# vribeiro1/artspeech

Measured on AMD Instinct MI355X. Metric: articulator-frames/sec (fwd+bwd), higher is better.
Workload: dtype f32

## Files before the change

artspeech_amd/csrc/artspeech.hip:

```cpp
#include <stdlib.h>

#include <algorithm>
#include <mutex>
#include <vector>

#include "gemm_internal.h"
#include "rowops.h"

namespace {

constexpr int D = AS_HEAD_HIDDEN;
constexpr int64_t SLAB_FLOATS = 16LL << 20;
constexpr int64_t SLAB2_FLOATS = 28LL << 20;

struct Carve {
    int64_t off = 0;
    int64_t take(int64_t n) {
        const int64_t o = off;
        off += as_round_up(n, 64);
        return o;
    }
};

struct HeadWs {
// ... 115 lines not shown
    as_gemm g{};
    g.A = A; g.B = Bm; g.C = C; g.M = M; g.N = N; g.K = K;
    g.a_i = 1; g.a_k = lda; g.b_j = 1; g.b_k = ldb; g.ldc = ldc;
    g.batch = batch; g.a_batch = ab; g.b_batch = bb; g.c_batch = cb; g.b_kshift = kshift; g.b_kT = kT; g.b_kshift_batch = kshift_batch;
    g.splitk_ws = slab; g.splitk_ws_floats = SLAB_FLOATS; g.colsum = colsum; g.colsum_batch = csb; g.cu_budget = cu_budget;
    return as_gemm_f32(&g, st);
}

int head_fold(const as_dims& d, const as_layout& L, const float* P, int64_t rows, float* ws, hipStream_t st) {
    const int A = d.n_art, H = d.hidden, O = 2 * d.n_samp;
    const HeadWs w = head_ws(d, rows);
    AS_STEP("head.fold", st, as_fold(P + L.w1, P + L.ln1_g, P + L.ln1_b, P + L.b1, ws + w.w1f, ws + w.b1f, A, D, H, st));
    AS_STEP("head.fold", st, as_fold(P + L.w2, P + L.ln2_g, P + L.ln2_b, P + L.b2, ws + w.w2f, ws + w.b2f, A, D, D, st));
    AS_STEP("head.fold", st, as_fold(P + L.w3, P + L.ln3_g, P + L.ln3_b, P + L.b3, ws + w.w3f, ws + w.b3f, A, O, D, st, (int)as_round_up(O, 32)));
    {
        const int Opad = (int)as_round_up(O, 32), Hp = (int)as_round_up(H, 32);
        auto up = [&](int64_t off) { return reinterpret_cast<uint16_t*>(ws + off); };
        as_planes_job j[6] = {
            {ws + w.w1f, H, 1, (long)D * H, A, D, H, D, Hp, up(w.w1p)},
            {ws + w.w2f, D, 1, (long)D * D, A, D, D, D, D, up(w.w2p)},
            {ws + w.w3f, D, 1, (long)Opad * D, A, O, D, (int)as_round_up(O, OUT_BN), D, up(w.w3p)},
            {ws + w.w2f, 1, D, (long)D * D, A, D, D, D, D, up(w.w2tp)},
            {ws + w.w3f, 1, D, (long)Opad * D, A, D, O, D, Opad, up(w.w3tp)},
            {ws + w.w1f, 1, H, 0, 1, H, A * D, (int)as_round_up(H, 128), A * D, up(w.w1tp)},
        };
        AS_STEP("head.planes", st, as_emit_planes(j, 6, st));
    }
    return 0;
}

struct Criterion { const float* tgt; long tgt_T; const int* lengths; int T; float scale; float* loss; float* dout; };

int head_fwd_impl(const as_dims& d, const as_layout& L, const float* P, const float* x, int64_t rows, float* out, float* ws,
                  hipStream_t st, const Criterion* crit = nullptr) {
    (void)P;
    const int A = d.n_art, H = d.hidden, O = 2 * d.n_samp;
    const HeadWs w = head_ws(d, rows);
    const int R = (int)rows;
    AS_STEP("head.norm0", st, as_normalize_fwd(x, ws + w.xhat, ws + w.rstd0, rows, H, st));
    const long AD = (long)A * D;
    const int Opad = (int)as_round_up(O, 32);
    unsigned long long* bits1 = reinterpret_cast<unsigned long long*>(ws + w.bits1);
    unsigned long long* bits2 = reinterpret_cast<unsigned long long*>(ws + w.bits2);
    as_lin l1{};
    l1.A = ws + w.xhat; l1.lda = H; l1.a_batch = 0;
    l1.B = ws + w.w1f; l1.ldb = H; l1.b_batch = (long)D * H; l1.b_kc = 1;
    l1.C = ws + w.r1hat; l1.ldc = AD; l1.c_batch = D;
    l1.bias = ws + w.b1f; l1.bias_batch = D;
    l1.M = R; l1.N = D; l1.K = H; l1.batch = A; l1.epi = 1;
    l1.rstd = ws + w.rstd1; l1.bits = bits1;
    const uint16_t* w1p = reinterpret_cast<const uint16_t*>(ws + w.w1p);
    const uint16_t* w2p = reinterpret_cast<const uint16_t*>(ws + w.w2p);
    if (H % 32 == 0) {
        l1.Bp = w1p; l1.bp_rows = D; l1.bp_batch = as_planes_batch_stride(D, H); l1.bp_plane = A * l1.bp_batch;
    }
    int took;
    bool crit_done = false;
    {
        AS_PROF("head.gemm1", st);
        took = as_lin_try(&l1, st);
        AS_REQUIRE(took >= 0, took, "head gemm1: launch failed");
    }
    if (!took) {
        AS_STEP("head.gemm1", st, gemm_nt(ws + w.xhat, H, ws + w.w1f, H, ws + w.r1, AD, ws + w.b1f, R, A * D, H, 1, st));
        AS_STEP("head.norm1", st, as_normalize_fwd(ws + w.r1, ws + w.r1hat, ws + w.rstd1, rows * A, D, st, bits1));
    }
    as_lin l2 = l1;
    l2.A = ws + w.r1hat; l2.lda = AD; l2.a_batch = D;
    l2.B = ws + w.w2f; l2.ldb = D; l2.b_batch = (long)D * D;
    l2.C = ws + w.r2hat; l2.bias = ws + w.b2f;
    l2.K = D; l2.rstd = ws + w.rstd2; l2.bits = bits2;
    l2.Bp = w2p; l2.bp_rows = D; l2.bp_batch = as_planes_batch_stride(D, D); l2.bp_plane = A * l2.bp_batch;
// ... 17 lines not shown
        AS_PROF("head.gemm3", st);
        as_lin_out lo{};
        lo.A = ws + w.r2hat; lo.lda = AD; lo.a_batch = D;
        lo.B = ws + w.w3f; lo.ldb = D; lo.b_batch = (long)Opad * D; lo.b_rows = Opad;
        lo.bias = ws + w.b3f; lo.bias_batch = O;
        lo.out = out; lo.ldo = (long)A * O; lo.o_batch = O;
        lo.M = R; lo.N = O; lo.K = D; lo.batch = A;
        lo.Bp = reinterpret_cast<const uint16_t*>(ws + w.w3p); lo.bp_rows = (int)as_round_up(O, OUT_BN);
        lo.bp_batch = as_planes_batch_stride(lo.bp_rows, D); lo.bp_plane = A * lo.bp_batch;
        int n_part = 0;
        if (crit) {
            lo.tgt = crit->tgt; lo.tgt_T = crit->tgt_T; lo.lengths = crit->lengths; lo.T = crit->T; lo.scale = crit->scale;
            lo.dout = crit->dout; lo.partial = ws + w.lpart; lo.partial_capacity = w.lpart_n; lo.loss = crit->loss;
        }
        took = as_lin_out_try(&lo, &n_part, st);
        AS_REQUIRE(took >= 0, took, "head gemm3: launch failed");
        if (took && crit && n_part > 0) AS_TRY(as_loss_final(ws + w.lpart, n_part, crit->scale, crit->loss, st));
        crit_done = took && crit;
        if (!took) {
            took = as_lin_try(&l3, st);
            AS_REQUIRE(took >= 0, took, "head gemm3: launch failed");
        }
    }
    if (!took)
        AS_STEP("head.gemm3", st, gemm_nt(ws + w.r2hat, AD, ws + w.w3f, D, out, (long)A * O, ws + w.b3f, R, O, D, 2, st, A, D,
                       (long)Opad * D, O, O));
    if (crit && !crit_done) {
        AS_STEP("loss", st, as_euclid_masked_fwd_bwd_presigmoid(out, crit->tgt, crit->tgt_T, crit->lengths, (int32_t)(rows / crit->T), crit->T, A,
                                                               d.n_samp, crit->scale, crit->loss, crit->dout, ws + w.lpart, st));
    }
    return 0;
}

int head_bwd_dx(const as_dims& d, const as_layout& L, const float* P, const float* out, const float* dout, int64_t rows,
                float* dx, const float* relu_src, float* ws, hipStream_t st, bool presig = false) {
    (void)L; (void)P;
    const int A = d.n_art, H = d.hidden, O = 2 * d.n_samp;
    const HeadWs w = head_ws(d, rows);
    const int R = (int)rows;
    const long AD = (long)A * D, AO = (long)A * O;
    const float* dpre3 = presig ? dout : ws + w.dpre3;
    if (!presig) AS_STEP("headb.sigmoid", st, as_sigmoid_bwd(out, dout, ws + w.dpre3, rows * AO, st));
    const int Opad = (int)as_round_up(O, 32);
    const unsigned long long* bits1 = reinterpret_cast<const unsigned long long*>(ws + w.bits1);
    const unsigned long long* bits2 = reinterpret_cast<const unsigned long long*>(ws + w.bits2);
    as_lin b3{};
    b3.A = dpre3; b3.lda = AO; b3.a_batch = O;
    b3.B = ws + w.w3f; b3.ldb = D; b3.b_batch = (long)Opad * D; b3.b_kc = 0;
    b3.C = ws + w.dz2; b3.ldc = AD; b3.c_batch = D;
    b3.M = R; b3.N = D; b3.K = Opad; b3.ka_valid = O; b3.batch = A; b3.epi = 2;
    b3.xhat = ws + w.r2hat; b3.ldx = AD; b3.x_batch = D; b3.rstd_in = ws + w.rstd2; b3.bits_in = bits2;
    b3.Bp = reinterpret_cast<const uint16_t*>(ws + w.w3tp); b3.bp_rows = D; b3.bp_batch = as_planes_batch_stride(D, Opad);
    b3.bp_plane = A * b3.bp_batch;
    int took;
    {
        AS_PROF("headb.dx3", st);
        took = as_lin_try(&b3, st);
        AS_REQUIRE(took >= 0, took, "head dx3: launch failed");
    }
    if (!took) {
        AS_STEP("headb.dx3", st, gemm_nn(dpre3, AO, ws + w.w3f, D, ws + w.dz2, AD, R, D, O, st, A, O, (long)Opad * D, D));
        AS_STEP("headb.norm2", st, as_normalize_bwd(ws + w.dz2, ws + w.r2hat, ws + w.rstd2, nullptr, ws + w.dz2, rows * A, D, st, bits2));
    }
    as_lin b2 = b3;
    b2.A = ws + w.dz2; b2.lda = AD; b2.a_batch = D;
    b2.B = ws + w.w2f; b2.b_batch = (long)D * D;
    b2.C = ws + w.dz1; b2.K = D; b2.ka_valid = D;
    b2.xhat = ws + w.r1hat; b2.rstd_in = ws + w.rstd1; b2.bits_in = bits1;
    b2.Bp = reinterpret_cast<const uint16_t*>(ws + w.w2tp); b2.bp_batch = as_planes_batch_stride(D, D); b2.bp_plane = A * b2.bp_batch;
    {
        AS_PROF("headb.dx2", st);
        took = as_lin_try(&b2, st);
        AS_REQUIRE(took >= 0, took, "head dx2: launch failed");
    }
    if (!took) {
        AS_STEP("headb.dx2", st, gemm_nn(ws + w.dz2, AD, ws + w.w2f, D, ws + w.dz1, AD, R, D, D, st, A, D, (long)D * D, D));
        AS_STEP("headb.norm1", st, as_normalize_bwd(ws + w.dz1, ws + w.r1hat, ws + w.rstd1, nullptr, ws + w.dz1, rows * A, D, st, bits1));
    }
    int dx1_slabs = 0;
    if (H <= 256 && H % 4 == 0) {
        as_lin l{};
        l.A = ws + w.dz1; l.lda = AD;
        l.Bp = reinterpret_cast<const uint16_t*>(ws + w.w1tp); l.bp_rows = (int)as_round_up(H, 128);
        l.bp_batch = as_planes_batch_stride(l.bp_rows, (int)AD); l.bp_plane = l.bp_batch;
        l.C = ws + w.slab; l.ldc = H;
        l.M = R; l.N = H; l.K = (int)AD; l.batch = 1;
        const int want = (int)std::max<int64_t>(1, std::min<int64_t>(8, 512 / std::max(1, as_cdiv(R, 64))));
        const int slabs = as_lin_plain_s6_slabs((int)AD, want);
        if ((int64_t)slabs * R * H <= SLAB_FLOATS) {
            AS_PROF("headb.dx1", st);
            const int took1 = as_lin_plain_s6(&l, want, (long)R * H, st);
            AS_REQUIRE(took1 >= 0, took1, "head dx1: launch failed");
            if (took1) dx1_slabs = slabs;
        }
    }
    if (!dx1_slabs)
        AS_STEP("headb.dx1", st, gemm_nn(ws + w.dz1, AD, ws + w.w1f, H, ws + w.dxhat, H, R, H, (int)AD, st, 1, 0, 0, 0, ws + w.slab));
    AS_STEP("headb.norm0", st, as_normalize_bwd(dx1_slabs ? ws + w.slab : ws + w.dxhat, ws + w.xhat, ws + w.rstd0, relu_src, dx, rows, H, st, nullptr,
                                                 dx1_slabs ? dx1_slabs : 1, (long)R * H));
    return 0;
}

struct TrunkJob { const float* dz; const float* y; float* dW; float* db; int H; };

int head_bwd_dw(const as_dims& d, const as_layout& L, const float* P, int64_t rows, float* G, float* ws, float* slab,
                hipStream_t st, const float* dpre3_in = nullptr, int cu_budget = 0, long slab_floats = SLAB_FLOATS,
                const TrunkJob* trunk = nullptr, int part = 0, int unfold_layers = -1) {
    const int A = d.n_art, H = d.hidden, O = 2 * d.n_samp;
    const HeadWs w = head_ws(d, rows);
    const int R = (int)rows;
    const long AD = (long)A * D, AO = (long)A * O;
    const float* dpre3 = dpre3_in ? dpre3_in : ws + w.dpre3;
    as_wgrad_job jobs[4] = {};
    as_gemm& g3 = jobs[0].g;
    g3.A = dpre3; g3.a_i = 1; g3.a_k = AO; g3.a_batch = O; g3.M = O;
    g3.B = ws + w.r2hat; g3.b_j = 1; g3.b_k = AD; g3.b_batch = D; g3.N = D;
    g3.C = ws + w.dw3f; g3.ldc = D; g3.c_batch = (long)O * D; g3.K = R; g3.batch = A;
    g3.colsum = G + L.b3; g3.colsum_batch = O;
    as_gemm& g1 = jobs[1].g;
    g1 = g3;
    g1.A = ws + w.xhat; g1.a_k = H; g1.a_batch = 0; g1.M = H;
    g1.B = ws + w.dz1;
    g1.C = ws + w.dw1f; g1.ldc = H; g1.c_batch = (long)D * H;
    g1.colsum = nullptr; g1.colsum_batch = 0;
    jobs[1].colsum_b = G + L.b1; jobs[1].colsum_b_batch = D; jobs[1].c_trans = 1;
    as_wgrad_job job2{};
    as_gemm& g2 = job2.g;
    g2 = g3;
    g2.A = ws + w.dz2; g2.a_k = AD; g2.a_batch = D; g2.M = D;
    g2.B = ws + w.r1hat;
// ... 221 lines not shown

extern "C" int as_artspeech_fwd(const as_dims* d, const float* P, const int64_t* tokens, int64_t tok_stride,
                                const int32_t* lengths, int32_t B, int32_t T, float* out, float* ws, int32_t train,
                                const as_opts* opts, void* stream) {
    AS_TRY(check_dims(d, "as_artspeech_fwd"));
    const float pdrop = (opts && train) ? opts->gru_dropout : 0.f;
    AS_REQUIRE(pdrop >= 0.f && pdrop < 1.f, AS_ERR_BAD_ARG, "as_artspeech_fwd: dropout %g not in [0, 1)", (double)pdrop);
    AS_REQUIRE(P && tokens && out && ws && B > 0 && T > 0 && tok_stride >= T, AS_ERR_BAD_ARG, "as_artspeech_fwd: bad argument");
    AS_REQUIRE(d->simple || lengths, AS_ERR_BAD_ARG, "as_artspeech_fwd: lengths required for the GRU model");
    AS_REQUIRE((int64_t)B * T < (1LL << 31), AS_ERR_BAD_ARG, "as_artspeech_fwd: B*T too large");
    hipStream_t st = (hipStream_t)stream;
    as_layout L;
    AS_TRY(as_artspeech_layout(d, &L));
    const ModelWs w = model_ws(*d, B, T);
    const int V = d->vocab, E = d->embed, H = d->hidden, R = B * T;
    StreamState* sd = d->simple ? nullptr : side_for(st);
    const bool late = opts && opts->fold_wait_event;
    if (late) {
        const hipError_t e = hipStreamWaitEvent(sd ? sd->side : st, (hipEvent_t)opts->fold_wait_event, 0);
        AS_REQUIRE(e == hipSuccess, (int)e, "as_artspeech_fwd: cannot wait for fold_wait_event: %s", hipGetErrorString(e));
    }
    if (sd) {
        if (!late) AS_TRY(fork_to(st, sd->side, sd->fork[0]));
        AS_TRY(head_fold(*d, L, P, R, ws + w.head, sd->side));
        AS_TRY(as_count_bad_tokens(tokens, tok_stride, T, R, V, reinterpret_cast<int*>(ws + w.tokflag), sd->side));
        if (hipEventRecord(sd->join, sd->side) != hipSuccess) {
            as_set_error("as_artspeech_fwd: event record failed");
            return AS_ERR_BAD_ARG;
        }
    } else {
        AS_TRY(head_fold(*d, L, P, R, ws + w.head, st));
        AS_TRY(as_count_bad_tokens(tokens, tok_stride, T, R, V, reinterpret_cast<int*>(ws + w.tokflag), st));
    }
    if (!d->simple) {
        if ((long)V * E <= 16384 && ((size_t)4 * E + 64 * ((size_t)E + 1)) * sizeof(float) <= 65536)
            AS_STEP("gru.table0", st, as_token_table(P + L.embedding, P + L.w_ih[0], P + L.b_ih[0], V, 6 * H, E, ws + w.tab0, st));
        else
            AS_STEP("gru.table0", st, gemm_nt(P + L.embedding, E, P + L.w_ih[0], E, ws + w.tab0, 6 * H, P + L.b_ih[0], V, 6 * H, E, 0, st));
        AS_STEP("gru.fwd_l0", st, as_gru_bidir_fwd_tokens(ws + w.tab0, tokens, tok_stride, V, P + L.w_hh[0], P + L.b_hh[0], lengths, B, T, H, ws + w.y0,
                                train ? ws + w.g0 : nullptr, st));
        const float* l1_in = ws + w.y0;
        if (pdrop > 0.f) {
            AS_STEP("gru.dropout", st, as_dropout(ws + w.y0, ws + w.y0d, (long)R * 2 * H, pdrop, opts->dropout_seed, st));
            l1_in = ws + w.y0d;
        }
        AS_STEP("gru.xproj1", st, gemm_nt(l1_in, 2 * H, P + L.w_ih[1], 2 * H, ws + w.xp1, 6 * H, P + L.b_ih[1], R, 6 * H, 2 * H, 0, st));
        AS_STEP("gru.fwd_l1", st, as_gru_bidir_fwd(ws + w.xp1, nullptr, 0, P + L.w_hh[1], P + L.b_hh[1], lengths, B, T, H, ws + w.y1,
                                train ? ws + w.g1 : nullptr, st));
        AS_STEP("trunk.linear", st, gemm_nt(ws + w.y1, 2 * H, P + L.lin_w, 2 * H, ws + w.lin, H, P + L.lin_b, R, H, 2 * H, 1, st));
    } else if (pdrop > 0.f) {
        AS_TRY(as_gather_rows(P + L.embedding, tokens, tok_stride, T, R, E, ws + w.y0, st, V));
        AS_TRY(as_dropout(ws + w.y0, ws + w.y0, (long)R * E, pdrop, opts->dropout_seed, st));
        AS_TRY(gemm_nt(ws + w.y0, E, P + L.lin_w, E, ws + w.lin, H, P + L.lin_b, R, H, E, 1, st));
    } else {
        AS_TRY(gemm_nt(P + L.embedding, E, P + L.lin_w, E, ws + w.tab0, H, P + L.lin_b, V, H, E, 1, st));
        AS_TRY(as_gather_rows(ws + w.tab0, tokens, tok_stride, T, R, H, ws + w.lin, st, V));
    }
    if (sd && hipStreamWaitEvent(st, sd->join, 0) != hipSuccess) {
        as_set_error("as_artspeech_fwd: stream wait failed");
        return AS_ERR_BAD_ARG;
    }
    if (opts && opts->loss_targets) {
        AS_REQUIRE(train && lengths && opts->loss_out && opts->loss_dout && opts->loss_tgt_T >= T, AS_ERR_BAD_ARG,
                   "as_artspeech_fwd: fused criterion needs train, lengths, loss_out, loss_dout and loss_tgt_T >= T");
        const Criterion crit{opts->loss_targets, (long)opts->loss_tgt_T, lengths, T, opts->loss_scale, opts->loss_out, opts->loss_dout};
        return head_fwd_impl(*d, L, P, ws + w.lin, R, out, ws + w.head, st, &crit);
    }
    return head_fwd_impl(*d, L, P, ws + w.lin, R, out, ws + w.head, st);
}

extern "C" int as_artspeech_dw2(const as_dims* d, const float* P, int32_t B, int32_t T, float* G, float* ws, void* stream) {
    AS_TRY(check_dims(d, "as_artspeech_dw2"));
    AS_REQUIRE(!d->simple && P && G && ws && B > 0 && T > 0, AS_ERR_BAD_ARG, "as_artspeech_dw2: bad argument");
    as_layout L;
    AS_TRY(as_artspeech_layout(d, &L));
    const ModelWs w = model_ws(*d, B, T);
    const HeadWs hw = head_ws(*d, (int64_t)B * T);
    float* hws = ws + w.head;
    return head_bwd_dw(*d, L, P, (int64_t)B * T, G, hws, hws + hw.slab2, (hipStream_t)stream, nullptr, 192, SLAB2_FLOATS, nullptr, 2, 2);
}

extern "C" int as_artspeech_bwd(const as_dims* d, const float* P, const int64_t* tokens, int64_t tok_stride,
                                const int32_t* lengths, int32_t B, int32_t T, const float* out, const float* dout, float* G,
                                float* ws, const as_opts* opts, void* stream) {
    AS_TRY(check_dims(d, "as_artspeech_bwd"));
    const float pdrop = opts ? opts->gru_dropout : 0.f;
    AS_REQUIRE(pdrop >= 0.f && pdrop < 1.f, AS_ERR_BAD_ARG, "as_artspeech_bwd: bad dropout option");
    AS_REQUIRE(P && tokens && out && dout && G && ws && B > 0 && T > 0 && tok_stride >= T, AS_ERR_BAD_ARG,
               "as_artspeech_bwd: bad argument");
    AS_REQUIRE(d->simple || lengths, AS_ERR_BAD_ARG, "as_artspeech_bwd: lengths required for the GRU model");
    hipStream_t st = (hipStream_t)stream;
    as_layout L;
    AS_TRY(as_artspeech_layout(d, &L));
    const ModelWs w = model_ws(*d, B, T);
    const HeadWs hw = head_ws(*d, (int64_t)B * T);
    const int V = d->vocab, E = d->embed, H = d->hidden, R = B * T;
    float* slab = ws + w.head + hw.slab;
    float* slab2 = ws + w.head + hw.slab2;
    float* dzlin = ws + w.head + hw.dxhat;
    float* hws = ws + w.head;
    const bool presig = opts && opts->dout_presigmoid;
    const float* dpre3 = presig ? dout : nullptr;
    AS_TRY(head_bwd_dx(*d, L, P, out, dout, R, dzlin, ws + w.lin, hws, st, presig));
    AS_REQUIRE(!(d->simple && opts && opts->defer_dw2), AS_ERR_UNSUPPORTED, "as_artspeech_bwd: defer_dw2 is for the GRU model");
    if (d->simple) {
        AS_TRY(head_bwd_dw(*d, L, P, R, G, hws, slab, st, dpre3));
        AS_TRY(record_heads_done(st, st));
        if (pdrop > 0.f) {
            AS_TRY(gemm_tn(dzlin, H, ws + w.y0, E, G + L.lin_w, E, H, E, R, st, slab, G + L.lin_b, 0));
            AS_TRY(gemm_nn(dzlin, H, P + L.lin_w, E, ws + w.dy0, E, R, E, H, st));
            AS_TRY(as_dropout(ws + w.dy0, ws + w.dy0, (long)R * E, pdrop, opts->dropout_seed, st));
            AS_TRY(as_token_segsum(ws + w.dy0, tokens, tok_stride, T, R, E, V, G + L.embedding, st, slab, SLAB_FLOATS));
            return 0;
        }
        AS_TRY(as_token_segsum(dzlin, tokens, tok_stride, T, R, H, V, ws + w.dtab0, st, slab, SLAB_FLOATS));
        AS_TRY(gemm_tn(ws + w.dtab0, H, P + L.embedding, E, G + L.lin_w, E, H, E, V, st, slab, G + L.lin_b, 0));
        AS_TRY(gemm_nn(ws + w.dtab0, H, P + L.lin_w, E, G + L.embedding, E, V, E, H, st));
        return 0;
    }
    StreamState* sd = side_for(st);
    hipStream_t s2 = sd ? sd->side : st;
    float* sl2 = sd ? slab2 : slab;
    hipStream_t s3 = (sd && sd->side2) ? sd->side2 : s2;
    float* sl3 = (sd && sd->side2) ? ws + w.head + hw.slab3 : sl2;
    hipStreamCaptureStatus cap_ = hipStreamCaptureStatusNone;
    const bool capturing = hipStreamIsCapturing(st, &cap_) != hipSuccess || cap_ != hipStreamCaptureStatusNone;
    const bool plain_forks = as_profile_active() || capturing;
    if (sd && !plain_forks) as_stop_event_set(sd->fork[0]);
    AS_STEP("trunkb.dx", st, gemm_nn(dzlin, H, P + L.lin_w, 2 * H, ws + w.dy1, 2 * H, R, 2 * H, H, st));
    if (sd) AS_TRY(fork_after(st, s2, sd->fork[0], plain_forks ? sd->fork[0] : as_stop_event_take()));
    AS_STEP("gru.bwd_l1", st, as_gru_bidir_bwd(ws + w.dy1, ws + w.y1, ws + w.g1, P + L.w_hh[1], lengths, B, T, H, ws + w.dgi1, ws + w.dgh1, st));
    const int side_cus = sd ? 192 : 0;
    const TrunkJob trunk{dzlin, ws + w.y1, G + L.lin_w, G + L.lin_b, H};
    const bool defer = opts && opts->defer_dw2;
    const bool two_parts = sd != nullptr || defer;
    AS_TRY(head_bwd_dw(*d, L, P, R, G, hws, sl2, s2, dpre3, side_cus, sd ? SLAB2_FLOATS : SLAB_FLOATS, &trunk, two_parts ? 1 : 0,
                       defer ? 5 : -1));
    if (!two_parts || defer) AS_TRY(record_heads_done(st, s2));
    const bool fork1_armed = sd && !plain_forks && !(pdrop > 0.f);
    if (fork1_armed) as_stop_event_set(sd->fork[1]);
    AS_STEP("grub.dx1", st, gemm_nn(ws + w.dgi1, 6 * H, P + L.w_ih[1], 2 * H, ws + w.dy0, 2 * H, R, 2 * H, 6 * H, st, 1, 0, 0, 0, slab));
    const hipEvent_t fork1_left = as_stop_event_take();
    if (pdrop > 0.f)
        AS_STEP("gru.dropout", st, as_dropout(ws + w.dy0, ws + w.dy0, (long)R * 2 * H, pdrop, opts->dropout_seed, st));
    if (sd) AS_TRY(fork_after(st, s2, sd->fork[1], fork1_armed ? fork1_left : sd->fork[1]));
    if (s3 != s2) {
        const hipError_t e = hipStreamWaitEvent(s3, sd->fork[1], 0);
        AS_REQUIRE(e == hipSuccess, (int)e, "as_artspeech_bwd: stream wait failed: %s", hipGetErrorString(e));
    }
    const int tok_sums = V <= T && as_gru_bwd_tokens_fits(V, H, T);
    if (sd && !plain_forks) as_stop_event_set(s3 != s2 ? sd->fork2[2] : sd->fork[2]);
    if (tok_sums) {
        AS_PROF("gru.bwd_l0", st);
        const int rc = as_gru_bidir_bwd_tokens(ws + w.dy0, ws + w.y0, ws + w.g0, P + L.w_hh[0], lengths, B, T, H, ws + w.dgh0, tokens,
                                               tok_stride, V, ws + w.dgi0, st);
        AS_REQUIRE(rc == 1, rc < 0 ? rc : AS_ERR_UNSUPPORTED, "gru.bwd_l0: launch failed");
    } else {
        AS_STEP("gru.bwd_l0", st, as_gru_bidir_bwd(ws + w.dy0, ws + w.y0, ws + w.g0, P + L.w_hh[0], lengths, B, T, H, ws + w.dgi0, ws + w.dgh0, st));
    }
    const hipEvent_t fork2_left = (sd && !plain_forks) ? as_stop_event_take() : (sd ? (s3 != s2 ? sd->fork2[2] : sd->fork[2]) : nullptr);
    if (two_parts && !defer) {
        AS_TRY(head_bwd_dw(*d, L, P, R, G, hws, sl2, s2, dpre3, side_cus, sd ? SLAB2_FLOATS : SLAB_FLOATS, nullptr, 2));
        AS_TRY(record_heads_done(st, s2));
    }
    AS_STEP("grub.dw_ih1", s2, gemm_tn(ws + w.dgi1, 6 * H, pdrop > 0.f ? ws + w.y0d : ws + w.y0, 2 * H, G + L.w_ih[1], 2 * H, 6 * H, 2 * H, R, s2, sl2, G + L.b_ih[1], 0));
    AS_STEP("grub.dw_hh", s3, gemm_tn(ws + w.dgh1, 6 * H, ws + w.y1, 2 * H, G + L.w_hh[1], H, 3 * H, H, R, s3, sl3, G + L.b_hh[1], 3 * H, 2,
                   3 * H, H, 3L * H * H, -1, T, 2));
    if (sd && s3 != s2) AS_TRY(fork_to(s2, s3, sd->join));
    hipStream_t s_hh = tok_sums ? st : s3, s_emb = tok_sums ? s3 : st;
    float* sl_hh = tok_sums ? slab : sl3;
    if (sd) AS_TRY(fork_after(st, s3, s3 != s2 ? sd->fork2[2] : sd->fork[2], fork2_left));
    AS_STEP("grub.dw_hh", s_hh, gemm_tn(ws + w.dgh0, 6 * H, ws + w.y0, 2 * H, G + L.w_hh[0], H, 3 * H, H, R, s_hh, sl_hh, G + L.b_hh[0], 3 * H, 2,
                   3 * H, H, 3L * H * H, -1, T, 2));
    if (tok_sums)
        AS_STEP("grub.segsum", s_emb, as_sum_partials(ws + w.dgi0, (long)V * 6 * H, B, ws + w.dtab0, s_emb));
    else
        AS_STEP("grub.segsum", s_emb, as_token_segsum(ws + w.dgi0, tokens, tok_stride, T, R, 6 * H, V, ws + w.dtab0, s_emb, slab, SLAB_FLOATS));
    if (E <= 256 && V <= 128 && (6 * H) % 16 == 0) {
        AS_STEP("grub.dw_ih0", s_emb, as_emb_grads(ws + w.dtab0, P + L.embedding, P + L.w_ih[0], V, 6 * H, E, G + L.w_ih[0], G + L.b_ih[0],
                                                G + L.embedding, s_emb));
    } else {
        float* sl_e = tok_sums ? sl3 : slab;
        AS_STEP("grub.dw_ih0", s_emb, gemm_tn(ws + w.dtab0, 6 * H, P + L.embedding, E, G + L.w_ih[0], E, 6 * H, E, V, s_emb, sl_e, G + L.b_ih[0], 0));
        AS_STEP("grub.demb", s_emb, gemm_nn(ws + w.dtab0, 6 * H, P + L.w_ih[0], E, G + L.embedding, E, V, E, 6 * H, s_emb, 1, 0, 0, 0, sl_e));
    }
    if (sd && s3 != s2) {
        AS_TRY(fork_to(s3, st, sd->join2));
    } else if (sd) {
        AS_TRY(fork_to(s2, st, sd->join));
    }
    return 0;
}
```

artspeech_amd/csrc/error.cpp:

```cpp
#include <stdarg.h>
#include <stdio.h>
#include <stdlib.h>
#include <string.h>

#include <atomic>

#include "artspeech_hip.h"

static thread_local char g_err[512] = "";

void as_set_error(const char* fmt, ...) {
    va_list ap;
    va_start(ap, fmt);
    vsnprintf(g_err, sizeof g_err, fmt, ap);
    va_end(ap);
}

extern "C" const char* as_last_error(void) { return g_err; }
extern "C" const char* as_version(void) { return "artspeech_hip 0.1.0"; }
extern "C" const char* as_arch(void) { return "gfx950"; }

static std::atomic<int> g_arith{-1};

int as_matrix_arith() {
    int m = g_arith.load(std::memory_order_relaxed);
    if (m < 0) {
        const char* e = getenv("ARTSPEECH_MATRIX_ARITH");
        m = (e && (!strcmp(e, "fp32") || !strcmp(e, "0"))) ? 0 : 1;
        g_arith.store(m, std::memory_order_relaxed);
    }
    return m;
}
extern "C" void as_set_matrix_arith(int32_t mode) { g_arith.store(mode ? 1 : 0, std::memory_order_relaxed); }
extern "C" int32_t as_get_matrix_arith(void) { return as_matrix_arith(); }

static thread_local void* g_stop_event = nullptr;
void as_stop_event_set_raw(void* ev) { g_stop_event = ev; }
void* as_stop_event_take_raw() {
    void* e = g_stop_event;
    g_stop_event = nullptr;
    return e;
}
```

artspeech_amd/csrc/gemm_f32.hip:

```cpp
#include <cstdlib>
#include <cstring>
#include <mutex>
#include <vector>

#include <hip/hip_ext.h>

#include "gemm_internal.h"

typedef float f32x16 __attribute__((ext_vector_type(16)));

namespace {

constexpr int BK = 32;

struct GemmK {
    const float* A; const float* B; float* C; const float* bias;
    int M, N, K;
    long a_i, a_k, b_j, b_k, ldc;
    long a_batch, b_batch, c_batch, bias_batch;
    int act, accumulate, b_kshift, b_kT, b_kshift_batch;
    int a_vec, b_vec;
    int splitk, kchunk, batch;
    int xcd_chunks;
    int xcd_panels;
// ... 555 lines not shown
        const bool more = work < total;
        if (more) {
            w = decode(work);
            tile_load<BM, true, true>(ra, w.A, g.a_i, 1, w.m0, 0, g.M, g.K, true, 0, 0, tid);
            tile_load<BN, true, true>(rb, w.B, g.b_j, 1, w.n0, 0, g.N, g.K, true, 0, 0, tid);
        }
        const float* bias = g.bias ? g.bias + (g.bias_off ? g.bias_off[bz] : (long)bz * g.bias_batch) : nullptr;
        const bool whole = m0 + BM <= g.M;
        float* c0 = C + (long)(m0 + wm * WM + 4 * lh) * g.ldc + n0 + wn * WN + l31;
#pragma unroll
        for (int j = 0; j < TN; ++j) {
            const int col = n0 + wn * WN + j * 32 + l31;
            if (col >= g.N) continue;
            const float bj = bias ? bias[col] : 0.f;
#pragma unroll
            for (int i = 0; i < TM; ++i)
#pragma unroll
                for (int r = 0; r < 16; ++r) {
                    const int rr = i * 32 + (r & 3) + 8 * (r >> 2);
                    if (!whole && m0 + wm * WM + 4 * lh + rr >= g.M) continue;
                    float v = acc[i][j][r] + bj;
                    if (g.act == 1) v = as_relu(v);
                    else if (g.act == 2) v = as_sigmoid(v);
                    else if (g.act == 3) v = 0.5f * v * (1.0f + erff(v * 0.70710678118654752440f));
                    float* c = c0 + (long)rr * g.ldc + j * 32;
                    if (g.accumulate) v += *c;
                    *c = v;
                }
        }
        if (!more) break;
    }
}

__global__ __launch_bounds__(256) void splitk_reduce_kernel(GemmK g) {
    const int ncs = g.colsum ? 1 : 0;
    const long W = g.N + ncs;
    const long per = (long)g.M * W;
    const long total = (long)g.batch * per;
    const long stride = (long)gridDim.x * 256;
    for (long idx = (long)blockIdx.x * 256 + threadIdx.x; idx < total; idx += stride) {
        float s = 0.f;
        for (int k = 0; k < g.splitk; ++k) s += g.slab[(long)k * total + idx];
        const long bz = idx / per, rem = idx - bz * per;
        const long row = rem / W;
        const int col = (int)(rem - row * W);
        if (col < g.N) {
            float* c = g.C + bz * g.c_batch + row * g.ldc + col;
            *c = g.accumulate ? *c + s : s;
        } else {
            g.colsum[bz * g.colsum_batch + row] = s;
        }
    }
}

__global__ __launch_bounds__(256) void splitk_reduce4_kernel(GemmK g) {
    __shared__ float part[3][64];
    const int ncs = g.colsum ? 1 : 0;
    const long W = g.N + ncs;
    const long per = (long)g.M * W;
    const long total = (long)g.batch * per;
    const int q = threadIdx.x >> 6, i = threadIdx.x & 63;
    const long idx = (long)blockIdx.x * 64 + i;
    const long src = idx < total ? idx : total - 1;
    float s = 0.f;
    for (int k = q; k < g.splitk; k += 4) s += g.slab[(long)k * total + src];
    if (q > 0) part[q - 1][i] = s;
// ... 14 lines not shown
template <typename Kern>
int resident_blocks(Kern kern) {
    int per_cu = 0, dev = 0, cus = 0;
    if (hipOccupancyMaxActiveBlocksPerMultiprocessor(&per_cu, kern, 256, 0) != hipSuccess || per_cu < 1) per_cu = 1;
    if (hipGetDevice(&dev) != hipSuccess || hipDeviceGetAttribute(&cus, hipDeviceAttributeMultiprocessorCount, dev) != hipSuccess || cus < 1)
        cus = 256;
    return per_cu * cus;
}

constexpr int COUNTERS = 8192;
int* counters_for(hipStream_t st) {
    struct Slot { int dev; hipStream_t st; int* p; };
    static std::mutex mu;
    static std::vector<Slot> slots;
    int dev = 0;
    if (hipGetDevice(&dev) != hipSuccess) return nullptr;
    std::lock_guard<std::mutex> lock(mu);
    for (const Slot& s : slots)
        if (s.dev == dev && s.st == st) return s.p;
    if (slots.size() >= 64) return nullptr;
    hipStreamCaptureStatus cap = hipStreamCaptureStatusNone;
    if (hipStreamIsCapturing(st, &cap) != hipSuccess || cap != hipStreamCaptureStatusNone) return nullptr;
    int* p = nullptr;
    if (hipMalloc(&p, COUNTERS * sizeof(int)) != hipSuccess) return nullptr;
    if (hipMemsetAsync(p, 0, COUNTERS * sizeof(int), st) != hipSuccess) { (void)hipFree(p); return nullptr; }
    slots.push_back({dev, st, p});
    return p;
}

}
int* as_arrival_counter(hipStream_t st) {
    int* p = counters_for(st);
    return p ? p + (COUNTERS - 1) : nullptr;
}
namespace {

template <int BM, int BN>
int launch(const GemmK& k, int batch, bool a_kc, bool b_kc, hipStream_t st) {
    const long work = (long)as_cdiv(k.M, BM) * as_cdiv(k.N, BN) * k.splitk * batch;
    dim3 block(256);
    const bool fast = k.a_vec && k.b_vec && (a_kc ? k.K % 4 == 0 : k.M % 4 == 0) && (b_kc ? k.K % 4 == 0 : k.N % 4 == 0);
    hipEvent_t stop_ev = (k.splitk == 1 || k.counters != nullptr) ? as_stop_event_take() : nullptr;
#define AS_GEMM_LAUNCH(AK, BK_, F)                                                                   \
    do {                                                                                             \
        static const int slots = resident_blocks(gemm_f32_kernel<BM, BN, AK, BK_, F>);               \
        const dim3 grid((unsigned)(work < slots ? work : slots));                                    \
        if (stop_ev) hipExtLaunchKernelGGL((gemm_f32_kernel<BM, BN, AK, BK_, F>), grid, block, 0, st, nullptr, stop_ev, 0, k); \
        else hipLaunchKernelGGL((gemm_f32_kernel<BM, BN, AK, BK_, F>), grid, block, 0, st, k);       \
    } while (0)
    if (k.res || k.mask_bits || k.relu_bits || k.k_seg > 0 || k.k_tri != 0) {
#define AS_GEMM_LAUNCH_EXT(AK, BK_)                                                                    \
    do {                                                                                               \
        static const int slots = resident_blocks(gemm_f32_kernel<BM, BN, AK, BK_, true, true>);        \
        const dim3 grid((unsigned)(work < slots ? work : slots));                                      \
        hipLaunchKernelGGL((gemm_f32_kernel<BM, BN, AK, BK_, true, true>), grid, block, 0, st, k);     \
    } while (0)
        if constexpr (BM == BN) {
            if (a_kc && b_kc) AS_GEMM_LAUNCH_EXT(true, true);
            else if (a_kc) AS_GEMM_LAUNCH_EXT(true, false);
            else if (!b_kc) AS_GEMM_LAUNCH_EXT(false, false);
            else AS_REQUIRE(false, AS_ERR_BAD_ARG, "as_gemm_f32: the extended operands have no kernel for a strided A with a contiguous B");
        } else {
            AS_REQUIRE(false, AS_ERR_BAD_ARG, "as_gemm_f32: the extended operands need a square tile");
        }
#undef AS_GEMM_LAUNCH_EXT
    } else if (fast) {
// ... 166 lines not shown
```

artspeech_amd/csrc/gemm_internal.h:

```cpp
#pragma once
#include "as_common.h"

int as_wgrad_try(const as_gemm* g, hipStream_t st);
struct as_wgrad_job {
    as_gemm g;
    float* colsum_b; long colsum_b_batch;
    int c_trans;
};
int as_wgrad_multi(const as_wgrad_job* jobs, int n, float* slab, long slab_floats, int cu_budget, hipStream_t st, bool exact = false);

enum { AS_ARITH_FP32 = 0, AS_ARITH_BF16X6 = 1 };
int as_matrix_arith();

struct as_planes_job {
    const float* B; long n_stride, k_stride, batch_stride;
    int batch, N, K, rows_pad, Kpad;
    uint16_t* out;
};
int as_emit_planes(const as_planes_job* jobs, int n, hipStream_t st);
static inline long as_planes_batch_stride(int rows_pad, int Kpad) { return (long)(Kpad / 16) * rows_pad * 16; }
static inline long as_planes_floats(int batch, int rows_pad, int Kpad) { return 3 * batch * as_planes_batch_stride(rows_pad, Kpad) / 2; }

int as_gemm_s6_nt(const float* A, long lda, long a_batch, const float* B, long ldb, long b_batch, const float* bias, long bias_batch, float* C,
                  long ldc, long c_batch, int M, int N, int K, int batch, int act, hipStream_t st);
int as_gemm_s6_nt_ext(const as_gemm* g, hipStream_t st);
template <int N> struct IC2 { static constexpr int value = N; };

void as_stop_event_set_raw(void* ev);
void* as_stop_event_take_raw();
inline void as_stop_event_set(hipEvent_t ev) { as_stop_event_set_raw((void*)ev); }
inline hipEvent_t as_stop_event_take() { return (hipEvent_t)as_stop_event_take_raw(); }

struct as_lin {
    const float* A; long lda, a_batch;
    const float* B; long ldb, b_batch; int b_kc;
    const uint16_t* Bp; long bp_plane, bp_batch; int bp_rows;
    float* C; long ldc, c_batch;
    const float* bias; long bias_batch;
    int M, N, K, ka_valid, batch, act, epi;
    float* rstd; unsigned long long* bits;
    const float* xhat; long ldx, x_batch; const float* rstd_in; const unsigned long long* bits_in;
    int tile_rows;
};
int as_lin_try(const as_lin* a, hipStream_t st);
int as_lin_plain_s6(const as_lin* a, int ksplit, long c_split, hipStream_t st);
static inline int as_lin_plain_s6_slabs(int K, int ksplit) {
    if (ksplit < 1) ksplit = 1;
    const int kchunk = (int)as_round_up(as_cdiv(K, ksplit), 32);
    return as_cdiv(K, kchunk);
}

struct as_lin_out {
    const float* A; long lda, a_batch;
    const float* B; long ldb, b_batch; int b_rows;
    const float* bias; long bias_batch;
    float* out; long ldo, o_batch;
    int M, N, K, batch;
    const float* tgt; long tgt_T; const int* lengths; int T; float scale;
    float* dout; float* partial; long partial_capacity;
    const uint16_t* Bp; long bp_plane, bp_batch; int bp_rows;
    float* loss;
};
int as_lin_out_try(const as_lin_out* a, int* n_partials, hipStream_t st);
int* as_arrival_counter(hipStream_t st);
int as_loss_final(const float* partial, int n, float scale, float* loss, hipStream_t st);

bool as_gru_bwd_tokens_fits(int32_t V, int32_t H, int32_t T);
int as_gru_bidir_bwd_tokens(const float* dy, const float* y, const float* gates, const float* w_hh, const int32_t* lengths,
                            int32_t B, int32_t T, int32_t H, float* dgh, const int64_t* tokens, int64_t tok_stride, int32_t V,
                            float* part, hipStream_t st);
int as_gru_bidir_fwd_tokens(const float* table, const int64_t* tokens, int64_t tok_stride, int32_t V, const float* w_hh,
                            const float* b_hh, const int32_t* lengths, int32_t B, int32_t T, int32_t H, float* y, float* gates,
                            hipStream_t st);
int as_count_bad_tokens(const int64_t* tokens, long tok_stride, int T, long rows, int V, int* count, hipStream_t st);
int as_sum_partials(const float* part, long n, int chunks, float* out, hipStream_t st);
```

Before: 6.448 million.

## Fuse trunk linear with head layer norm in forward and backward

Adds two new kernels. The forward one computes the trunk linear layer with ReLU and then layer-normalizes the same rows inside one kernel, so the head's separate normalize launch is skipped. The backward one sums the split-K slabs, applies the layer-norm and ReLU backward, and multiplies by the trunk weight to get the input gradient, replacing a normalize-bwd launch plus a GEMM. This cuts kernel launches and global round-trips of the intermediate rows. The cost is specialized kernels that only handle H=128, plus extra stop-event plumbing through an RAII helper, with an environment-variable switch to fall back to the old path.

```diff
diff --git a/artspeech_amd/csrc/artspeech.hip b/artspeech_amd/csrc/artspeech.hip
--- a/artspeech_amd/csrc/artspeech.hip
+++ b/artspeech_amd/csrc/artspeech.hip
@@ -171,12 +171,12 @@
 struct Criterion { const float* tgt; long tgt_T; const int* lengths; int T; float scale; float* loss; float* dout; };
 
 int head_fwd_impl(const as_dims& d, const as_layout& L, const float* P, const float* x, int64_t rows, float* out, float* ws,
-                  hipStream_t st, const Criterion* crit = nullptr) {
+                  hipStream_t st, const Criterion* crit = nullptr, bool norm0_done = false) {
     (void)P;
     const int A = d.n_art, H = d.hidden, O = 2 * d.n_samp;
     const HeadWs w = head_ws(d, rows);
     const int R = (int)rows;
-    AS_STEP("head.norm0", st, as_normalize_fwd(x, ws + w.xhat, ws + w.rstd0, rows, H, st));
+    if (!norm0_done) AS_STEP("head.norm0", st, as_normalize_fwd(x, ws + w.xhat, ws + w.rstd0, rows, H, st));
     const long AD = (long)A * D;
     const int Opad = (int)as_round_up(O, 32);
     unsigned long long* bits1 = reinterpret_cast<unsigned long long*>(ws + w.bits1);
@@ -260,8 +260,9 @@
     return 0;
 }
 
+struct Norm0Left { int max_slabs; const float* dy; int n_slab; long slab_stride; };
 int head_bwd_dx(const as_dims& d, const as_layout& L, const float* P, const float* out, const float* dout, int64_t rows,
-                float* dx, const float* relu_src, float* ws, hipStream_t st, bool presig = false) {
+                float* dx, const float* relu_src, float* ws, hipStream_t st, bool presig = false, Norm0Left* left = nullptr) {
     (void)L; (void)P;
     const int A = d.n_art, H = d.hidden, O = 2 * d.n_samp;
     const HeadWs w = head_ws(d, rows);
@@ -324,6 +325,12 @@
     }
     if (!dx1_slabs)
         AS_STEP("headb.dx1", st, gemm_nn(ws + w.dz1, AD, ws + w.w1f, H, ws + w.dxhat, H, R, H, (int)AD, st, 1, 0, 0, 0, ws + w.slab));
+    if (left && std::max(dx1_slabs, 1) <= left->max_slabs) {
+        left->dy = dx1_slabs ? ws + w.slab : ws + w.dxhat;
+        left->n_slab = std::max(dx1_slabs, 1);
+        left->slab_stride = (long)R * H;
+        return 0;
+    }
     AS_STEP("headb.norm0", st, as_normalize_bwd(dx1_slabs ? ws + w.slab : ws + w.dxhat, ws + w.xhat, ws + w.rstd0, relu_src, dx, rows, H, st, nullptr,
                                                  dx1_slabs ? dx1_slabs : 1, (long)R * H));
     return 0;
@@ -611,6 +618,7 @@
         AS_TRY(head_fold(*d, L, P, R, ws + w.head, st));
         AS_TRY(as_count_bad_tokens(tokens, tok_stride, T, R, V, reinterpret_cast<int*>(ws + w.tokflag), st));
     }
+    bool norm0_done = false;
     if (!d->simple) {
         if ((long)V * E <= 16384 && ((size_t)4 * E + 64 * ((size_t)E + 1)) * sizeof(float) <= 65536)
             AS_STEP("gru.table0", st, as_token_table(P + L.embedding, P + L.w_ih[0], P + L.b_ih[0], V, 6 * H, E, ws + w.tab0, st));
@@ -626,7 +634,16 @@
         AS_STEP("gru.xproj1", st, gemm_nt(l1_in, 2 * H, P + L.w_ih[1], 2 * H, ws + w.xp1, 6 * H, P + L.b_ih[1], R, 6 * H, 2 * H, 0, st));
         AS_STEP("gru.fwd_l1", st, as_gru_bidir_fwd(ws + w.xp1, nullptr, 0, P + L.w_hh[1], P + L.b_hh[1], lengths, B, T, H, ws + w.y1,
                                 train ? ws + w.g1 : nullptr, st));
-        AS_STEP("trunk.linear", st, gemm_nt(ws + w.y1, 2 * H, P + L.lin_w, 2 * H, ws + w.lin, H, P + L.lin_b, R, H, 2 * H, 1, st));
+        if (!(as_parent_launches() & AS_PARENT_TRUNK_FWD)) {
+            AS_PROF("trunk.linear", st);
+            const HeadWs hw = head_ws(*d, R);
+            const int took = as_trunk_norm_fwd(ws + w.y1, 2 * H, P + L.lin_w, 2 * H, P + L.lin_b, ws + w.lin, ws + w.head + hw.xhat,
+                                               ws + w.head + hw.rstd0, R, H, 2 * H, st);
+            AS_REQUIRE(took >= 0, took, "trunk linear: launch failed");
+            norm0_done = took != 0;
+        }
+        if (!norm0_done)
+            AS_STEP("trunk.linear", st, gemm_nt(ws + w.y1, 2 * H, P + L.lin_w, 2 * H, ws + w.lin, H, P + L.lin_b, R, H, 2 * H, 1, st));
     } else if (pdrop > 0.f) {
         AS_TRY(as_gather_rows(P + L.embedding, tokens, tok_stride, T, R, E, ws + w.y0, st, V));
         AS_TRY(as_dropout(ws + w.y0, ws + w.y0, (long)R * E, pdrop, opts->dropout_seed, st));
@@ -643,9 +660,9 @@
         AS_REQUIRE(train && lengths && opts->loss_out && opts->loss_dout && opts->loss_tgt_T >= T, AS_ERR_BAD_ARG,
                    "as_artspeech_fwd: fused criterion needs train, lengths, loss_out, loss_dout and loss_tgt_T >= T");
         const Criterion crit{opts->loss_targets, (long)opts->loss_tgt_T, lengths, T, opts->loss_scale, opts->loss_out, opts->loss_dout};
-        return head_fwd_impl(*d, L, P, ws + w.lin, R, out, ws + w.head, st, &crit);
-    }
-    return head_fwd_impl(*d, L, P, ws + w.lin, R, out, ws + w.head, st);
+        return head_fwd_impl(*d, L, P, ws + w.lin, R, out, ws + w.head, st, &crit, norm0_done);
+    }
+    return head_fwd_impl(*d, L, P, ws + w.lin, R, out, ws + w.head, st, nullptr, norm0_done);
 }
 
 extern "C" int as_artspeech_dw2(const as_dims* d, const float* P, int32_t B, int32_t T, float* G, float* ws, void* stream) {
@@ -680,7 +697,10 @@
     float* hws = ws + w.head;
     const bool presig = opts && opts->dout_presigmoid;
     const float* dpre3 = presig ? dout : nullptr;
-    AS_TRY(head_bwd_dx(*d, L, P, out, dout, R, dzlin, ws + w.lin, hws, st, presig));
+    Norm0Left left{8, nullptr, 0, 0};
+    const bool trunk_fused = !d->simple && !(as_parent_launches() & AS_PARENT_TRUNK_BWD) &&
+                             as_trunk_norm_bwd_fits(H, 2 * H, P + L.lin_w, 2 * H, 1);
+    AS_TRY(head_bwd_dx(*d, L, P, out, dout, R, dzlin, ws + w.lin, hws, st, presig, trunk_fused ? &left : nullptr));
     AS_REQUIRE(!(d->simple && opts && opts->defer_dw2), AS_ERR_UNSUPPORTED, "as_artspeech_bwd: defer_dw2 is for the GRU model");
     if (d->simple) {
         AS_TRY(head_bwd_dw(*d, L, P, R, G, hws, slab, st, dpre3));
@@ -705,9 +725,18 @@
     hipStreamCaptureStatus cap_ = hipStreamCaptureStatusNone;
     const bool capturing = hipStreamIsCapturing(st, &cap_) != hipSuccess || cap_ != hipStreamCaptureStatusNone;
     const bool plain_forks = as_profile_active() || capturing;
-    if (sd && !plain_forks) as_stop_event_set(sd->fork[0]);
-    AS_STEP("trunkb.dx", st, gemm_nn(dzlin, H, P + L.lin_w, 2 * H, ws + w.dy1, 2 * H, R, 2 * H, H, st));
-    if (sd) AS_TRY(fork_after(st, s2, sd->fork[0], plain_forks ? sd->fork[0] : as_stop_event_take()));
+    {
+        AsStopEventArm arm((sd && !plain_forks) ? sd->fork[0] : nullptr);
+        if (left.dy) {
+            AS_PROF("trunkb.dx", st);
+            const int took = as_trunk_norm_bwd(left.dy, left.n_slab, left.slab_stride, hws + hw.xhat, hws + hw.rstd0, ws + w.lin, P + L.lin_w,
+                                               2 * H, dzlin, ws + w.dy1, R, H, 2 * H, st);
+            AS_REQUIRE(took != 0, took < 0 ? took : AS_ERR_UNSUPPORTED, "trunk input gradient: launch failed");
+        } else {
+            AS_STEP("trunkb.dx", st, gemm_nn(dzlin, H, P + L.lin_w, 2 * H, ws + w.dy1, 2 * H, R, 2 * H, H, st));
+        }
+        if (sd) AS_TRY(fork_after(st, s2, sd->fork[0], plain_forks ? sd->fork[0] : arm.take()));
+    }
     AS_STEP("gru.bwd_l1", st, as_gru_bidir_bwd(ws + w.dy1, ws + w.y1, ws + w.g1, P + L.w_hh[1], lengths, B, T, H, ws + w.dgi1, ws + w.dgh1, st));
     const int side_cus = sd ? 192 : 0;
     const TrunkJob trunk{dzlin, ws + w.y1, G + L.lin_w, G + L.lin_b, H};
@@ -717,9 +746,12 @@
                        defer ? 5 : -1));
     if (!two_parts || defer) AS_TRY(record_heads_done(st, s2));
     const bool fork1_armed = sd && !plain_forks && !(pdrop > 0.f);
-    if (fork1_armed) as_stop_event_set(sd->fork[1]);
-    AS_STEP("grub.dx1", st, gemm_nn(ws + w.dgi1, 6 * H, P + L.w_ih[1], 2 * H, ws + w.dy0, 2 * H, R, 2 * H, 6 * H, st, 1, 0, 0, 0, slab));
-    const hipEvent_t fork1_left = as_stop_event_take();
+    hipEvent_t fork1_left = nullptr;
+    {
+        AsStopEventArm arm(fork1_armed ? sd->fork[1] : nullptr);
+        AS_STEP("grub.dx1", st, gemm_nn(ws + w.dgi1, 6 * H, P + L.w_ih[1], 2 * H, ws + w.dy0, 2 * H, R, 2 * H, 6 * H, st, 1, 0, 0, 0, slab));
+        fork1_left = arm.take();
+    }
     if (pdrop > 0.f)
         AS_STEP("gru.dropout", st, as_dropout(ws + w.dy0, ws + w.dy0, (long)R * 2 * H, pdrop, opts->dropout_seed, st));
     if (sd) AS_TRY(fork_after(st, s2, sd->fork[1], fork1_armed ? fork1_left : sd->fork[1]));
@@ -728,16 +760,19 @@
         AS_REQUIRE(e == hipSuccess, (int)e, "as_artspeech_bwd: stream wait failed: %s", hipGetErrorString(e));
     }
     const int tok_sums = V <= T && as_gru_bwd_tokens_fits(V, H, T);
-    if (sd && !plain_forks) as_stop_event_set(s3 != s2 ? sd->fork2[2] : sd->fork[2]);
-    if (tok_sums) {
-        AS_PROF("gru.bwd_l0", st);
-        const int rc = as_gru_bidir_bwd_tokens(ws + w.dy0, ws + w.y0, ws + w.g0, P + L.w_hh[0], lengths, B, T, H, ws + w.dgh0, tokens,
-                                               tok_stride, V, ws + w.dgi0, st);
-        AS_REQUIRE(rc == 1, rc < 0 ? rc : AS_ERR_UNSUPPORTED, "gru.bwd_l0: launch failed");
-    } else {
-        AS_STEP("gru.bwd_l0", st, as_gru_bidir_bwd(ws + w.dy0, ws + w.y0, ws + w.g0, P + L.w_hh[0], lengths, B, T, H, ws + w.dgi0, ws + w.dgh0, st));
-    }
-    const hipEvent_t fork2_left = (sd && !plain_forks) ? as_stop_event_take() : (sd ? (s3 != s2 ? sd->fork2[2] : sd->fork[2]) : nullptr);
+    hipEvent_t fork2_left = sd ? (s3 != s2 ? sd->fork2[2] : sd->fork[2]) : nullptr;
+    {
+        AsStopEventArm arm((sd && !plain_forks) ? fork2_left : nullptr);
+        if (tok_sums) {
+            AS_PROF("gru.bwd_l0", st);
+            const int rc = as_gru_bidir_bwd_tokens(ws + w.dy0, ws + w.y0, ws + w.g0, P + L.w_hh[0], lengths, B, T, H, ws + w.dgh0, tokens,
+                                                   tok_stride, V, ws + w.dgi0, st);
+            AS_REQUIRE(rc == 1, rc < 0 ? rc : AS_ERR_UNSUPPORTED, "gru.bwd_l0: launch failed");
+        } else {
+            AS_STEP("gru.bwd_l0", st, as_gru_bidir_bwd(ws + w.dy0, ws + w.y0, ws + w.g0, P + L.w_hh[0], lengths, B, T, H, ws + w.dgi0, ws + w.dgh0, st));
+        }
+        if (sd && !plain_forks) fork2_left = arm.take();
+    }
     if (two_parts && !defer) {
         AS_TRY(head_bwd_dw(*d, L, P, R, G, hws, sl2, s2, dpre3, side_cus, sd ? SLAB2_FLOATS : SLAB_FLOATS, nullptr, 2));
         AS_TRY(record_heads_done(st, s2));
diff --git a/artspeech_amd/csrc/error.cpp b/artspeech_amd/csrc/error.cpp
--- a/artspeech_amd/csrc/error.cpp
+++ b/artspeech_amd/csrc/error.cpp
@@ -41,3 +41,8 @@
     g_stop_event = nullptr;
     return e;
 }
+
+int as_parent_launches() {
+    const char* e = getenv("ARTSPEECH_PARENT_LAUNCHES");
+    return e ? atoi(e) : 0;
+}
diff --git a/artspeech_amd/csrc/gemm_f32.hip b/artspeech_amd/csrc/gemm_f32.hip
--- a/artspeech_amd/csrc/gemm_f32.hip
+++ b/artspeech_amd/csrc/gemm_f32.hip
@@ -611,6 +611,204 @@
     }
 }
 
+struct TrunkNormK {
+    const float* A; const float* B; const float* bias;
+    float* lin; float* xhat; float* rstd;
+    int M, N, K; long lda, ldb; float eps;
+};
+
+__global__ __launch_bounds__(256) void trunk_norm_fwd_kernel(TrunkNormK g) {
+    constexpr int BM = 32, BN = 128;
+    constexpr int LDT = BN + 8;
+    __shared__ __attribute__((aligned(16))) float sA[Img<BM, true>::size];
+    __shared__ __attribute__((aligned(16))) float sB[Img<BN, true>::size];
+    __shared__ float rows[BM * LDT];
+    const int tid = threadIdx.x, lane = tid & 63, wave = tid >> 6;
+    const int l31 = lane & 31, lh = lane >> 5;
+    const int m0 = blockIdx.x * BM;
+    float4 ra[BM / 32], rb[BN / 32];
+    tile_load<BM, true, true>(ra, g.A, g.lda, 1, m0, 0, g.M, g.K, true, 0, 0, tid);
+    tile_load<BN, true, true>(rb, g.B, g.ldb, 1, 0, 0, g.N, g.K, true, 0, 0, tid);
+    f32x16 acc;
+#pragma unroll
+    for (int r = 0; r < 16; ++r) acc[r] = 0.f;
+    const int nk = (g.K + BK - 1) / BK;
+    tile_store<BM, true>(sA, ra, tid);
+    tile_store<BN, true>(sB, rb, tid);
+    __syncthreads();
+    for (int kt = 0; kt < nk; ++kt) {
+        if (kt + 1 < nk) {
+            tile_load<BM, true, true>(ra, g.A, g.lda, 1, m0, (kt + 1) * BK, g.M, g.K, true, 0, 0, tid);
+            tile_load<BN, true, true>(rb, g.B, g.ldb, 1, 0, (kt + 1) * BK, g.N, g.K, true, 0, 0, tid);
+        }
+#pragma unroll
+        for (int kk = 0; kk < BK; kk += 2) {
+            const float av = frag<BM, true>(sA, l31, kk + lh);
+            const float bv = frag<BN, true>(sB, wave * 32 + l31, kk + lh);
+            acc = __builtin_amdgcn_mfma_f32_32x32x2f32(av, bv, acc, 0, 0, 0);
+        }
+        if (kt + 1 < nk) {
+            __syncthreads();
+            tile_store<BM, true>(sA, ra, tid);
+            tile_store<BN, true>(sB, rb, tid);
+            __syncthreads();
+        }
+    }
+    {
+        const int col = wave * 32 + l31;
+        const float bj = g.bias ? g.bias[col] : 0.f;
+#pragma unroll
+        for (int r = 0; r < 16; ++r) {
+            float v = acc[r] + bj;
+            v = as_relu(v);
+            rows[((r & 3) + 8 * (r >> 2) + 4 * lh) * LDT + col] = v;
+        }
+    }
+    __syncthreads();
+    const int D = g.N;
+#pragma unroll
+    for (int rr = 0; rr < BM / 4; ++rr) {
+        const int rl = wave + 4 * rr;
+        const long row = (long)m0 + rl;
+        if (row < g.M) {
+#pragma clang fp contract(off)
+            const float* xr = rows + rl * LDT;
+            float v[2];
+#pragma unroll
+            for (int c = 0; c < 2; ++c) {
+                const int i = lane + 64 * c;
+                v[c] = xr[i < D ? i : D - 1];
+            }
+            float* lo = g.lin + row * D;
+#pragma unroll
+            for (int c = 0; c < 2; ++c)
+                if (lane + 64 * c < D) lo[lane + 64 * c] = v[c];
+#pragma unroll
+            for (int c = 0; c < 2; ++c)
+                if (lane + 64 * c >= D) v[c] = 0.f;
+            const float s = (0.f + v[0]) + v[1];
+            const float mean = as_wave_sum(s) / D;
+#pragma unroll
+            for (int c = 0; c < 2; ++c) v[c] = lane + 64 * c < D ? v[c] - mean : 0.f;
+            const float q1 = v[1] * v[1];
+            const float q = __builtin_fmaf(v[0], v[0], q1);
+            const float rs = 1.0f / sqrtf(as_wave_sum(q) / D + g.eps);
+            float* o = g.xhat + row * D;
+#pragma unroll
+            for (int c = 0; c < 2; ++c) {
+                const int i = lane + 64 * c;
+                if (i < D) o[i] = v[c] * rs;
+            }
+            if (lane == 0) g.rstd[row] = rs;
+        }
+    }
+}
+
+constexpr int TRUNK_SLABS = 8;
+
+struct TrunkBwdK {
+    const float* dy; int n_slab; long slab_stride;
+    const float* xhat; const float* rstd; const float* relu_src;
+    const float* W; long ldw;
+    float* dz; float* dx;
+    int M, D, N;
+};
+
+__global__ __launch_bounds__(256, 1) void trunk_norm_bwd_kernel(TrunkBwdK g) {
+    constexpr int BM = 32, BD = 128, BN = 256, NKT = BD / BK;
+    constexpr int LDA = BD + 1;
+    __shared__ __attribute__((aligned(16))) float sB[Img<BN, false>::size];
+    __shared__ float sZ[BM * LDA];
+    const int tid = threadIdx.x, lane = tid & 63, wave = tid >> 6;
+    const int l31 = lane & 31, lh = lane >> 5;
+    const int m0 = blockIdx.x * BM;
+    float4 rb[NKT][BN / 32];
+#pragma unroll
+    for (int t = 0; t < NKT; ++t) tile_load<BN, false, true>(rb[t], g.W, 1, g.ldw, 0, t * BK, g.N, g.D, true, 0, 0, tid);
+    const int D = g.D;
+    {
+        constexpr int RW = BM / 4;
+        float gg[RW][2], h[RW][2], m[RW][2], part[RW][TRUNK_SLABS - 1][2], rs[RW];
+#pragma unroll
+        for (int rr = 0; rr < RW; ++rr) {
+            const long row = min((long)m0 + wave + 4 * rr, (long)g.M - 1);
+            const float* dyr = g.dy + row * D;
+#pragma unroll
+            for (int c = 0; c < 2; ++c) {
+                const int i = lane + 64 * c;
+                const int ic = i < D ? i : D - 1;
+                gg[rr][c] = dyr[ic];
+                h[rr][c] = g.xhat[row * D + ic];
+                m[rr][c] = g.relu_src[row * D + ic];
+#pragma unroll
+                for (int sl = 1; sl < TRUNK_SLABS; ++sl)
+                    part[rr][sl - 1][c] = dyr[min(sl, g.n_slab - 1) * g.slab_stride + ic];
+            }
+            rs[rr] = g.rstd[row];
+        }
+#pragma unroll
+        for (int rr = 0; rr < RW; ++rr) {
+#pragma clang fp contract(off)
+            const int rl = wave + 4 * rr;
+            const long row = (long)m0 + rl;
+#pragma unroll
+            for (int sl = 1; sl < TRUNK_SLABS; ++sl)
+#pragma unroll
+                for (int c = 0; c < 2; ++c) {
+                    const float sum = gg[rr][c] + part[rr][sl - 1][c];
+                    gg[rr][c] = sl < g.n_slab ? sum : gg[rr][c];
+                }
+#pragma unroll
+            for (int c = 0; c < 2; ++c)
+                if (lane + 64 * c >= D) gg[rr][c] = 0.f;
+            const float p0 = gg[rr][0] * h[rr][0], p1 = gg[rr][1] * h[rr][1];
+            const float s1 = (0.f + gg[rr][0]) + gg[rr][1];
+            const float s2 = (0.f + p0) + p1;
+            const float m1 = as_wave_sum(s1) / D, m2 = as_wave_sum(s2) / D;
+#pragma unroll
+            for (int c = 0; c < 2; ++c) {
+                const int i = lane + 64 * c;
+                const float t = gg[rr][c] - m1;
+                float v = rs[rr] * __builtin_fmaf(-h[rr][c], m2, t);
+                if (!(m[rr][c] > 0.f)) v = 0.f;
+                if (i < D) {
+                    sZ[rl * LDA + i] = v;
+                    if (row < g.M) g.dz[row * D + i] = v;
+                }
+            }
+        }
+    }
+    f32x16 acc[2];
+#pragma unroll
+    for (int j = 0; j < 2; ++j)
+#pragma unroll
+        for (int r = 0; r < 16; ++r) acc[j][r] = 0.f;
+#pragma unroll
+    for (int t = 0; t < NKT; ++t) {
+        if (t > 0) __syncthreads();
+        tile_store<BN, false>(sB, rb[t], tid);
+        __syncthreads();
+#pragma unroll
+        for (int kk = 0; kk < BK; kk += 2) {
+            const float av = sZ[l31 * LDA + t * BK + kk + lh];
+#pragma unroll
+            for (int j = 0; j < 2; ++j) {
+                const float bv = frag<BN, false>(sB, wave * 64 + j * 32 + l31, kk + lh);
+                acc[j] = __builtin_amdgcn_mfma_f32_32x32x2f32(av, bv, acc[j], 0, 0, 0);
+            }
+        }
+    }
+#pragma unroll
+    for (int j = 0; j < 2; ++j) {
+        const int col = wave * 64 + j * 32 + l31;
+#pragma unroll
+        for (int r = 0; r < 16; ++r) {
+            const long row = (long)m0 + (r & 3) + 8 * (r >> 2) + 4 * lh;
+            if (row < g.M) g.dx[row * g.N + col] = acc[j][r];
+        }
+    }
+}
+
 __global__ __launch_bounds__(256) void splitk_reduce_kernel(GemmK g) {
     const int ncs = g.colsum ? 1 : 0;
     const long W = g.N + ncs;
@@ -691,6 +889,39 @@
 int* as_arrival_counter(hipStream_t st) {
     int* p = counters_for(st);
     return p ? p + (COUNTERS - 1) : nullptr;
+}
+
+int as_trunk_norm_fwd(const float* A, long lda, const float* W, long ldw, const float* bias, float* lin, float* xhat, float* rstd,
+                      long M, int N, int K, hipStream_t st) {
+    auto al16 = [](const void* p) { return (reinterpret_cast<uintptr_t>(p) & 15) == 0; };
+    if (N != 128 || K < 1 || K % 4 || M < 1 || M >= (1L << 31) - 32 || lda % 4 || ldw % 4 || !al16(A) || !al16(W)) return 0;
+    TrunkNormK k{A, W, bias, lin, xhat, rstd, (int)M, N, K, lda, ldw, 1e-5f};
+    hipLaunchKernelGGL(trunk_norm_fwd_kernel, dim3((unsigned)as_cdiv(M, 32)), dim3(256), 0, st, k);
+    hipError_t e = hipGetLastError();
+    if (e != hipSuccess) {
+        as_set_error("as_trunk_norm_fwd: launch failed: %s", hipGetErrorString(e));
+        return -(int)e;
+    }
+    return 1;
+}
+
+bool as_trunk_norm_bwd_fits(int D, int N, const float* W, long ldw, int n_slab) {
+    return D == 128 && N == 256 && n_slab >= 1 && n_slab <= TRUNK_SLABS && ldw % 4 == 0 && (reinterpret_cast<uintptr_t>(W) & 15) == 0;
+}
+int as_trunk_norm_bwd(const float* dy, int n_slab, long slab_stride, const float* xhat, const float* rstd, const float* relu_src,
+                      const float* W, long ldw, float* dz, float* dx, long M, int D, int N, hipStream_t st) {
+    if (!as_trunk_norm_bwd_fits(D, N, W, ldw, n_slab) || !relu_src || M < 1 || M >= (1L << 31) - 32) return 0;
+    TrunkBwdK k{dy, n_slab, slab_stride, xhat, rstd, relu_src, W, ldw, dz, dx, (int)M, D, N};
+    const dim3 grid((unsigned)as_cdiv(M, 32)), block(256);
+    hipEvent_t stop_ev = as_stop_event_take();
+    if (stop_ev) hipExtLaunchKernelGGL(trunk_norm_bwd_kernel, grid, block, 0, st, nullptr, stop_ev, 0, k);
+    else hipLaunchKernelGGL(trunk_norm_bwd_kernel, grid, block, 0, st, k);
+    hipError_t e = hipGetLastError();
+    if (e != hipSuccess) {
+        as_set_error("as_trunk_norm_bwd: launch failed: %s", hipGetErrorString(e));
+        return -(int)e;
+    }
+    return 1;
 }
 namespace {
 
diff --git a/artspeech_amd/csrc/gemm_internal.h b/artspeech_amd/csrc/gemm_internal.h
--- a/artspeech_amd/csrc/gemm_internal.h
+++ b/artspeech_amd/csrc/gemm_internal.h
@@ -30,6 +30,16 @@
 void* as_stop_event_take_raw();
 inline void as_stop_event_set(hipEvent_t ev) { as_stop_event_set_raw((void*)ev); }
 inline hipEvent_t as_stop_event_take() { return (hipEvent_t)as_stop_event_take_raw(); }
+struct AsStopEventArm {
+    explicit AsStopEventArm(hipEvent_t ev) { if (ev) as_stop_event_set(ev); }
+    ~AsStopEventArm() { (void)as_stop_event_take_raw(); }
+    AsStopEventArm(const AsStopEventArm&) = delete;
+    AsStopEventArm& operator=(const AsStopEventArm&) = delete;
+    hipEvent_t take() { return as_stop_event_take(); }
+};
+
+enum { AS_PARENT_TRUNK_FWD = 1, AS_PARENT_TRUNK_BWD = 2 };
+int as_parent_launches();
 
 struct as_lin {
     const float* A; long lda, a_batch;
@@ -63,6 +73,11 @@
 };
 int as_lin_out_try(const as_lin_out* a, int* n_partials, hipStream_t st);
 int* as_arrival_counter(hipStream_t st);
+int as_trunk_norm_fwd(const float* A, long lda, const float* W, long ldw, const float* bias, float* lin, float* xhat, float* rstd,
+                      long M, int N, int K, hipStream_t st);
+bool as_trunk_norm_bwd_fits(int D, int N, const float* W, long ldw, int n_slab);
+int as_trunk_norm_bwd(const float* dy, int n_slab, long slab_stride, const float* xhat, const float* rstd, const float* relu_src,
+                      const float* W, long ldw, float* dz, float* dx, long M, int D, int N, hipStream_t st);
 int as_loss_final(const float* partial, int n, float scale, float* loss, hipStream_t st);
 
 bool as_gru_bwd_tokens_fits(int32_t V, int32_t H, int32_t T);
```

Measured after the change: 6.462 million (median of 6 runs). About the same (+0.2%).
